# xiangxiecrypto/tfhe-omr

Measured on AMD Instinct MI355X. Metric: detect-phase messages/sec + per-message latency, D=65536 at 1/2/4/8 MI355X, higher is better.
Workload: dtype f64

## Files before the change

tfhe-omr_amd/csrc/br2_fft.hpp:

```cpp
#pragma once

#include "exactness.hpp"
#include "fft1024.hpp"
#include "handoff.hpp"
#include "level2_common.hpp"

namespace omr {

__device__ __forceinline__ int key_pos(int t, int e) { return e * Fft1024::T + t; }


struct Digits2S {
  static constexpr int DW = 2;
  static_assert(LOGB2 == 7 && D2 == 6 && DROP2 == 8, "closed form written for the level-2 basis");
  __device__ static __forceinline__ void pack(double v, uint32_t (&pk)[DW]) {
    const double y = floor(__fma_rn(v, 1.0 / 256.0, 0.5)) + (17315143744.0 + 6755399441055744.0);
    const uint64_t b = __builtin_bit_cast(uint64_t, y);
    const uint32_t lo = (uint32_t)b, hi = (uint32_t)(b >> 32);
    pk[0] = lo ^ 0x102040u;
    pk[1] = __builtin_amdgcn_alignbit(hi, lo, 21) ^ 0x2040u;
  }
  static constexpr int TOP_WIDTH = 16;
  template <int H>
  __device__ static __forceinline__ double digit(const uint32_t (&pk)[DW], int j) {
    return (double)(int)__builtin_amdgcn_sbfe(pk[H], 7 * j, H == 1 && j == 2 ? TOP_WIDTH : 7);
  }
};

__device__ __forceinline__ double limb_acc(double acc, double lo, double hr) {
  using M = Mod<2>;
  const double x = acc + lo;
  const double hi = hr * LIMB;
  const double k = rint(__fma_rn(hr, LIMB * M::QINV, x * M::QINV));
  return canon_small<M>(__fma_rn(-k, M::Q, hi) + x);
}

constexpr int BR2_ROW = 4 * Fft1024::n;
__device__ __forceinline__ __amdgpu_buffer_rsrc_t bsk2_rsrc(const double2 *bskf) {
  constexpr uint32_t bytes = (uint32_t)((size_t)NI * 2 * D2 * BR2_ROW * sizeof(double2));
  return __builtin_amdgcn_make_buffer_rsrc(const_cast<double2 *>(bskf), 0, bytes, 0x00020000);
}
typedef unsigned br2_v4u __attribute__((ext_vector_type(4)));
__device__ __forceinline__ void br2f_load_block(double2 (&k)[Fft1024::E], __amdgpu_buffer_rsrc_t rsrc, int q, int o,
                                                int l, uint32_t t16) {
#pragma unroll
  for (int e = 0; e < Fft1024::E; ++e) {
    const uint32_t soff = (uint32_t)q * (uint32_t)(BR2_ROW * sizeof(double2)) +
                          (uint32_t)(((o * 2 + l) * Fft1024::n + e * Fft1024::T) * sizeof(double2));
    k[e] = __builtin_bit_cast(double2, __builtin_amdgcn_raw_buffer_load_b128(rsrc, t16, (int)soff, 0));
  }
}
__device__ __forceinline__ void br2f_load_half(double2 (&k)[2][Fft1024::E], __amdgpu_buffer_rsrc_t rsrc, int q,
                                               int o, uint32_t t16) {
  br2f_load_block(k[0], rsrc, q, o, 0, t16);
  br2f_load_block(k[1], rsrc, q, o, 1, t16);
}
__device__ __forceinline__ void br2f_mac(const double (&xr)[Fft1024::E], const double (&xi)[Fft1024::E],
                                         const double2 (&k)[2][Fft1024::E], double (&sr)[2][Fft1024::E],
                                         double (&si)[2][Fft1024::E]) {
#pragma unroll
  for (int l = 0; l < 2; ++l)
#pragma unroll
    for (int e = 0; e < Fft1024::E; ++e) {
      const double2 kv = k[l][e];
      sr[l][e] = __fma_rn(xr[e], kv.x, __fma_rn(-xi[e], kv.y, sr[l][e]));
      si[l][e] = __fma_rn(xr[e], kv.y, __fma_rn(xi[e], kv.x, si[l][e]));
    }
}
__device__ __forceinline__ void br2f_zero(double (&sr)[2][2][Fft1024::E], double (&si)[2][2][Fft1024::E]) {
#pragma unroll
  for (int o = 0; o < 2; ++o)
#pragma unroll
    for (int l = 0; l < 2; ++l)
#pragma unroll
      for (int e = 0; e < Fft1024::E; ++e) sr[o][l][e] = si[o][l][e] = 0.0;
}

__device__ __forceinline__ void br2f_digits(const double *acp, int a, int t,
                                            uint32_t (&pk)[2][Fft1024::E][Digits2S::DW]) {
  using F = Fft1024;
  using M = Mod<2>;
  constexpr int NN = N2;
#pragma unroll
  for (int h = 0; h < 2; ++h)
#pragma unroll
    for (int e = 0; e < F::E; ++e) {
      const int c = F::idx(0, t, e) + F::n * h;
      const uint32_t u = (uint32_t)(c - a) & (2 * NN - 1);
      const double v = acp[F::slot_stage(u & (NN - 1))];
      const uint32_t vh = (uint32_t)(__builtin_bit_cast(uint64_t, v) >> 32) ^ ((u & NN) << (31 - 11));
      const double rot = __builtin_bit_cast(double, (__builtin_bit_cast(uint64_t, v) & 0xffffffffull) |
                                                        ((uint64_t)vh << 32));
      Digits2S::pack(canon_small<M>(rot - acp[F::slot_stage(c)]), pk[h][e]);
      asm volatile("" : "+v"(pk[h][e][0]), "+v"(pk[h][e][1]));
    }
}

template <int W>
__device__ __forceinline__ void br2f_digit(const uint32_t (&pk)[2][Fft1024::E][Digits2S::DW], int j, int q, int nx,
                                           double (&sr)[2][2][Fft1024::E], double (&si)[2][2][Fft1024::E],
                                           double2 (&ka)[2][Fft1024::E], double2 (&kb)[2][Fft1024::E], double2 *X,
                                           __amdgpu_buffer_rsrc_t rsrc, uint32_t t16, int t, const double2 (&wc)[4][2]) {
  using F = Fft1024;
  constexpr int E = F::E;
  double xr[E], xi[E];
#pragma unroll
  for (int e = 0; e < E; ++e) {
    xr[e] = Digits2S::digit<W>(pk[0][e], j);
    xi[e] = Digits2S::digit<W>(pk[1][e], j);
  }
  constexpr int LE = 1;
  F::fwd(xr, xi, X, t, wc, [&]() {
    __builtin_amdgcn_s_setprio(2);
#pragma unroll
    for (int l = 0; l < LE; ++l) br2f_load_block(kb[l], rsrc, q, 1, l, t16);
  });
#pragma unroll
  for (int l = LE; l < 2; ++l) br2f_load_block(kb[l], rsrc, q, 1, l, t16);
#pragma unroll
  for (int o = 0; o < 2; ++o) {
    br2f_mac(xr, xi, o ? kb : ka, sr[o], si[o]);
    if (o == 0) br2f_load_half(ka, rsrc, nx, 0, t16);
  }
  __builtin_amdgcn_s_setprio(0);
}

template <bool G>
__device__ __forceinline__ void br2f_update(double *aco, const double (&sr)[2][Fft1024::E],
                                           const double (&si)[2][Fft1024::E], RoundGuard<G> &rg, int t) {
  using F = Fft1024;
#pragma unroll
  for (int e = 0; e < F::E; ++e)
#pragma unroll
    for (int h = 0; h < 2; ++h) {
      const double ylo = h ? si[0][e] : sr[0][e], yhi = h ? si[1][e] : sr[1][e];
      const double lo = rint(ylo), hr = rint(yhi);
      rg.note(ylo, lo);
      rg.note(yhi, hr);
      double &a = aco[F::slot_stage(F::idx(0, t, e) + F::n * h)];
      a = limb_acc(a, lo, hr);
    }
}

constexpr size_t BR2_LDS_X = 0, BR2_LDS_TWS = 4 * (size_t)Fft1024::n * sizeof(double2),
                 BR2_LDS_BYTES = BR2_LDS_TWS + (size_t)Fft1024::n * sizeof(double2);
struct Br2Lds {
  double2 *tws;
  double2 (*Xb)[Fft1024::n];
  double *acs;
};
__device__ __forceinline__ Br2Lds br2_lds(double2 *pool) {
  double2 *x = pool + BR2_LDS_X / sizeof(double2);
  return {pool + BR2_LDS_TWS / sizeof(double2), reinterpret_cast<double2(*)[Fft1024::n]>(x),
          reinterpret_cast<double *>(x + 2 * Fft1024::n)};
}

template <bool G>
__device__ __forceinline__ void br2f_trace(const Br2Lds &lds, const double2 *__restrict__ tkf,
                                           const double2 *__restrict__ twg, const DeviceTables &tb,
                                           RoundGuard<G> &rg, int t) {
  using F = Fft1024;
  using M = Mod<2>;
  constexpr int E = F::E, NN = N2;
  double *acs = lds.acs;
  double2(*Xb)[F::n] = lds.Xb;
  const double2 *tws = lds.tws;
  double2 wc[4][2];
  F::load_ct(wc, twg, t);
  static_assert(DT == 25 && TRACE_STEPS == 11, "trace geometry");
#pragma unroll
  for (int p = 0; p < 2; ++p)
#pragma unroll
    for (int h = 0; h < 2; ++h)
#pragma unroll
      for (int e = 0; e < E; ++e) {
        double &x = acs[p * NN + F::slot_stage(F::idx(0, t, e) + F::n * h)];
        x = canon<M>(mm<M>(x, NINV2));
      }
  constexpr uint32_t bytes = (uint32_t)((size_t)TRACE_STEPS * DT * BR2_ROW * sizeof(double2));
  const __amdgpu_buffer_rsrc_t rsrc = __builtin_amdgcn_make_buffer_rsrc(const_cast<double2 *>(tkf), 0, bytes, 0x00020000);
  const uint32_t t16 = (uint32_t)t * 16u;
#pragma unroll 1
  for (int k = 0; k < TRACE_STEPS; ++k) {
    const uint16_t *src = tb.trace_src + k * NN;
    double2 ka[2][E], kb[2][E];
    br2f_load_half(ka, rsrc, k * DT, 0, t16);
    __syncthreads();
    uint32_t pk[2][E][DigitsTrace::DW];
#pragma unroll
    for (int h = 0; h < 2; ++h)
#pragma unroll
      for (int e = 0; e < E; ++e) {
        const int sidx = src[F::idx(0, t, e) + F::n * h];
        const double v = sidx < NN ? acs[F::slot_stage(sidx)] : -acs[F::slot_stage(sidx - NN)];
        DigitsTrace::pack(v, pk[h][e]);
        asm volatile("" : "+v"(pk[h][e][0]), "+v"(pk[h][e][1]));
      }
    double sr[2][2][E], si[2][2][E];
    br2f_zero(sr, si);
#pragma unroll 1
    for (int d = 0; d < DT; ++d) {
      const int q = k * DT + d;
      double xr[E], xi[E];
#pragma unroll
      for (int e = 0; e < E; ++e) {
        xr[e] = DigitsTrace::get(pk[0][e], d);
        xi[e] = DigitsTrace::get(pk[1][e], d);
      }
      F::fwd(xr, xi, Xb[d & 1], t, wc, [&]() { br2f_load_block(kb[0], rsrc, q, 1, 0, t16); });
      br2f_load_block(kb[1], rsrc, q, 1, 1, t16);
#pragma unroll
      for (int o = 0; o < 2; ++o) {
        br2f_mac(xr, xi, o ? kb : ka, sr[o], si[o]);
        if (o == 0) br2f_load_half(ka, rsrc, d + 1 < DT ? q + 1 : q, 0, t16);
      }
    }
#pragma unroll
    for (int o = 0; o < 2; ++o)
#pragma unroll
      for (int l = 0; l < 2; ++l) F::inv(sr[o][l], si[o][l], Xb[l], tws, t);
    double sb[2][E];
    const uint16_t *srcb = src;
#pragma unroll
    for (int h = 0; h < 2; ++h)
#pragma unroll
      for (int e = 0; e < E; ++e) {
        const int sidx = srcb[F::idx(0, t, e) + F::n * h];
        sb[h][e] = sidx < NN ? acs[NN + F::slot_stage(sidx)] : -acs[NN + F::slot_stage(sidx - NN)];
      }
    __syncthreads();
#pragma unroll
    for (int e = 0; e < E; ++e)
#pragma unroll
      for (int h = 0; h < 2; ++h) {
        const int c = F::slot_stage(F::idx(0, t, e) + F::n * h);
        const double alo = h ? si[0][0][e] : sr[0][0][e], ahi = h ? si[0][1][e] : sr[0][1][e];
        const double blo = h ? si[1][0][e] : sr[1][0][e], bhi = h ? si[1][1][e] : sr[1][1][e];
        const double ral = rint(alo), rah = rint(ahi), rbl = rint(blo), rbh = rint(bhi);
        rg.note(alo, ral);
        rg.note(ahi, rah);
        rg.note(blo, rbl);
        rg.note(bhi, rbh);
        acs[c] = limb_acc(acs[c], ral, rah);
        acs[NN + c] = limb_acc(acs[NN + c] + sb[h][e], rbl, rbh);
      }
  }
}

template <bool G, bool FROM = false>
__device__ __forceinline__ void br2f_body(const uint32_t *__restrict__ lwe_int, const double2 *__restrict__ bskf,
                                          const double2 *__restrict__ twg, DeviceTables tb, uint64_t *__restrict__ out,
                                          unsigned long long *margin, double2 *pool, size_t item,
                                          const uint64_t *__restrict__ acc0 = nullptr) {
  using F = Fft1024;
  using M = Mod<2>;
  constexpr int E = F::E, NN = N2;
  static_assert(F::TW_LEN <= F::n, "the twiddle table's LDS doubles as the trace's NTT table");
  const Br2Lds lds = br2_lds(pool);
  double2 *tws = lds.tws;
  double2(*Xb)[F::n] = lds.Xb;
  double *acs = lds.acs;
  const int t = threadIdx.x;
  const uint32_t *lwe = lwe_int + item * (NI + 1);
  F::load_twiddles(tws, twg, t);
  if constexpr (FROM) {
    const uint64_t *a0 = acc0 + item * 2 * NN;
#pragma unroll
    for (int h = 0; h < 2; ++h)
#pragma unroll
      for (int e = 0; e < E; ++e) {
        const int c = F::idx(0, t, e) + F::n * h;
        acs[F::slot_stage(c)] = from_u64<M>(a0[c]);
        acs[NN + F::slot_stage(c)] = from_u64<M>(a0[NN + c]);
      }
  } else {
    const int b = (int)lwe[NI];
#pragma unroll
    for (int h = 0; h < 2; ++h)
#pragma unroll
      for (int e = 0; e < E; ++e) {
        const int c = F::idx(0, t, e) + F::n * h;
        acs[F::slot_stage(c)] = 0.0;
        acs[NN + F::slot_stage(c)] = acc2_init(tb.lut2, b, c);
      }
  }
  __syncthreads();
  double2 wc[4][2];
  F::load_ct(wc, twg, t);
  double2 ka[2][E], kb[2][E];
  const __amdgpu_buffer_rsrc_t rsrc = bsk2_rsrc(bskf);
  const uint32_t t16 = (uint32_t)t * 16u;
  RoundGuard<G> rg;
  int kq = -1;
#pragma unroll 1
  for (int i = 0; i < NI; ++i) {
    const int a = (int)__builtin_amdgcn_readfirstlane(lwe[i]) & (2 * NN - 1);
    if (a == 0) continue;
    const int q0 = i * 2 * D2;
    if (kq != q0) br2f_load_half(ka, rsrc, q0, 0, t16);
    kq = i + 1 < NI ? q0 + 2 * D2 : -1;
    wg_barrier_lds();
    double sr[2][2][E], si[2][2][E];
#pragma unroll
    for (int p = 0; p < 2; ++p) {
      uint32_t pk[2][E][Digits2S::DW];
      br2f_digits(acs + p * NN, a, t, pk);
      auto nxt = [&](int j, int w) {
        return q0 + (w == 0 ? p * D2 + j + 3
                            : (j + 1 < D2 / 2 ? p * D2 + j + 1 : (p == 0 ? D2 : (kq >= 0 ? 2 * D2 : 2 * D2 - 1))));
      };
      if (p == 0) br2f_zero(sr, si);
#pragma unroll 1
      for (int j = 0; j < D2 / 2; ++j) {
        br2f_digit<0>(pk, j, q0 + p * D2 + j, nxt(j, 0), sr, si, ka, kb, Xb[0], rsrc, t16, t, wc);
        br2f_digit<1>(pk, j, q0 + p * D2 + j + 3, nxt(j, 1), sr, si, ka, kb, Xb[1], rsrc, t16, t, wc);
      }
    }
#pragma unroll
    for (int o = 0; o < 2; ++o) {
#pragma unroll
      for (int l = 0; l < 2; ++l) F::inv(sr[o][l], si[o][l], Xb[l], tws, t);
      br2f_update<G>(acs + o * NN, sr[o], si[o], rg, t);
    }
  }
  rg.publish(margin);
  __syncthreads();
  uint64_t *o = out + item * 2 * NN;
#pragma unroll
  for (int p = 0; p < 2; ++p)
#pragma unroll
    for (int h = 0; h < 2; ++h)
#pragma unroll
      for (int e = 0; e < E; ++e) {
        const int c = F::idx(0, t, e) + F::n * h;
        o[p * NN + c] = to_u64<M>(acs[p * NN + F::slot_stage(c)]);
      }
}

template <bool G>
__device__ __forceinline__ void trace_fft_body(uint64_t *__restrict__ io, const double2 *__restrict__ tkf,
                                               const double2 *__restrict__ twg, DeviceTables tb,
                                               unsigned long long *margin) {
  using F = Fft1024;
  using M = Mod<2>;
  constexpr int E = F::E, NN = N2;
  __shared__ double2 pool[BR2_LDS_BYTES / sizeof(double2)];
  const Br2Lds lds = br2_lds(pool);
  double2 *tws = lds.tws;
  double *acs = lds.acs;
  const int t = threadIdx.x;
  uint64_t *o = io + (size_t)blockIdx.x * 2 * NN;
  F::load_twiddles(tws, twg, t);
#pragma unroll
  for (int p = 0; p < 2; ++p)
#pragma unroll
    for (int h = 0; h < 2; ++h)
#pragma unroll
      for (int e = 0; e < E; ++e) {
        const int c = F::idx(0, t, e) + F::n * h;
        acs[p * NN + F::slot_stage(c)] = from_u64<M>(o[p * NN + c]);
      }
  RoundGuard<G> rg;
  br2f_trace<G>(lds, tkf, twg, tb, rg, t);
  rg.publish(margin);
  __syncthreads();
  using NTT = WgNtt<M, BR2_T, BR2_E>;
  double ca[BR2_E], cb[BR2_E];
#pragma unroll
  for (int e = 0; e < BR2_E; ++e) {
    ca[e] = acs[F::slot_stage(t + e * BR2_T)];
    cb[e] = acs[NN + F::slot_stage(t + e * BR2_T)];
  }
  double *xch = reinterpret_cast<double *>(lds.Xb);
  double *tw = reinterpret_cast<double *>(tws);
  static_assert(NTT::LDS_DOUBLES * sizeof(double) <= 2 * F::n * sizeof(double2), "NTT exchange below ACC");
#pragma unroll
  for (int e = 0; e < BR2_E; ++e) tw[t + e * BR2_T] = tb.tw2[t + e * BR2_T];
  __syncthreads();
  NTT::fwd(ca, xch, tw, t);
  NTT::fwd(cb, xch, tw, t);
#pragma unroll
  for (int e = 0; e < BR2_E; ++e) {
    const int j = t * BR2_E + e;
    o[j] = to_u64<M>(canon<M>(ca[e]));
    o[NN + j] = to_u64<M>(canon<M>(cb[e]));
  }
}
#ifndef OMR_LEVEL2_PARTS_ONLY
__global__ __launch_bounds__(256, 2) void trace_fft_kernel(uint64_t *__restrict__ io, const double2 *__restrict__ tkf,
                                                           const double2 *__restrict__ twg, DeviceTables tb) {
  trace_fft_body<false>(io, tkf, twg, tb, nullptr);
}
__global__ __launch_bounds__(256, 2) void trace_fft_guard_kernel(uint64_t *__restrict__ io,
                                                                 const double2 *__restrict__ tkf,
                                                                 const double2 *__restrict__ twg, DeviceTables tb,
                                                                 unsigned long long *margin) {
  trace_fft_body<true>(io, tkf, twg, tb, margin);
}

__global__ __launch_bounds__(256, 2) void br2f_kernel(const uint32_t *__restrict__ lwe_int,
                                                      const double2 *__restrict__ bskf,
                                                      const double2 *__restrict__ twg, DeviceTables tb,
                                                      uint64_t *__restrict__ out) {
  __shared__ double2 pool[BR2_LDS_BYTES / sizeof(double2)];
  br2f_body<false>(lwe_int, bskf, twg, tb, out, nullptr, pool, blockIdx.x);
}
__global__ __launch_bounds__(256, 2) void br2f_guard_kernel(const uint32_t *__restrict__ lwe_int,
                                                            const double2 *__restrict__ bskf,
                                                            const double2 *__restrict__ twg, DeviceTables tb,
                                                            uint64_t *__restrict__ out, unsigned long long *margin) {
  __shared__ double2 pool[BR2_LDS_BYTES / sizeof(double2)];
  br2f_body<true>(lwe_int, bskf, twg, tb, out, margin, pool, blockIdx.x);
}
__global__ __launch_bounds__(256, 2) void br2f_from_kernel(const uint32_t *__restrict__ lwe_int,
                                                           const double2 *__restrict__ bskf,
                                                           const double2 *__restrict__ twg, DeviceTables tb,
                                                           uint64_t *__restrict__ out,
                                                           const uint64_t *__restrict__ acc0) {
  __shared__ double2 pool[BR2_LDS_BYTES / sizeof(double2)];
  br2f_body<false, true>(lwe_int, bskf, twg, tb, out, nullptr, pool, blockIdx.x, acc0);
}
__global__ __launch_bounds__(256, 2) void br2f_guard_from_kernel(const uint32_t *__restrict__ lwe_int,
                                                                 const double2 *__restrict__ bskf,
                                                                 const double2 *__restrict__ twg, DeviceTables tb,
                                                                 uint64_t *__restrict__ out,
                                                                 unsigned long long *margin,
                                                                 const uint64_t *__restrict__ acc0) {
  __shared__ double2 pool[BR2_LDS_BYTES / sizeof(double2)];
  br2f_body<true, true>(lwe_int, bskf, twg, tb, out, margin, pool, blockIdx.x, acc0);
}
#endif


constexpr int BR2Y_T = 2 * Fft1024::T;
constexpr int BR2Y_H = 4, BR2Y_PF = 2;

__device__ __forceinline__ void br2y_prefetch(const uint32_t *__restrict__ lwe_int, const double2 *__restrict__ bskf,
                                              const uint32_t *flags, int wid, int k) {
  constexpr int STEP_LINES = D2 * BR2_ROW * (int)sizeof(double2) / 64;
  constexpr int PER_THREAD = STEP_LINES / (BR2Y_H * BR2Y_T);
  static_assert(PER_THREAD * BR2Y_H * BR2Y_T == STEP_LINES, "helpers split a step's rows evenly");
  __shared__ int go;
  const int m = wid >> 1, r = wid & 1;
  const uint32_t *lwe = lwe_int + (size_t)m * (NI + 1);
  uint32_t acc = 0;
  int e = 0;
#pragma unroll 1
  for (int i = 0; i < NI; ++i) {
    const int a = (int)__builtin_amdgcn_readfirstlane(lwe[i]) & (2 * N2 - 1);
    if (a == 0) continue;
    if (threadIdx.x == 0) {
      int ok = 1, n = 0;
      while ((int)__hip_atomic_load(flags + wid, __ATOMIC_RELAXED, __HIP_MEMORY_SCOPE_AGENT) < e - BR2Y_PF) {
        if (++n == (1 << 16)) {
          ok = 0;
          break;
        }
        __builtin_amdgcn_s_sleep(2);
      }
      go = ok;
    }
    __syncthreads();
    if (!go) break;
    const char *rows = reinterpret_cast<const char *>(bskf + ((size_t)i * 2 * D2 + (size_t)r * D2) * BR2_ROW);
    uint32_t v[PER_THREAD];
#pragma unroll
    for (int u = 0; u < PER_THREAD; ++u)
      v[u] = *reinterpret_cast<const uint32_t *>(rows + (size_t)((u * BR2Y_H + k) * BR2Y_T + (int)threadIdx.x) * 64);
#pragma unroll
    for (int u = 0; u < PER_THREAD; ++u) acc ^= v[u];
    __syncthreads();
    ++e;
  }
  asm volatile("" ::"v"(acc));
}

#ifndef OMR_LEVEL2_PARTS_ONLY
__global__ __launch_bounds__(BR2Y_T, 1) void br2y_kernel(const uint32_t *__restrict__ lwe_int,
                                                         const double2 *__restrict__ bskf,
                                                         const double2 *__restrict__ twg, DeviceTables tb,
                                                         double *xg, uint32_t *flags, int *err,
                                                         uint64_t *__restrict__ out, int nmsg, int w8,
                                                         int allow_fast) {
#define OMR_BR2Y_FROM 0
#include "br2y_kernel_body.inc"
#undef OMR_BR2Y_FROM
}
#endif

}
```

tfhe-omr_amd/csrc/fft1024.hpp:

```cpp
#pragma once

#include "device_fft.hpp"

namespace omr {

struct Fft1024 {
  static constexpr int T = 256, E = 4, n = 1024, L = 10;
  static constexpr int TW_LEN = 3 * (4 + 16 + 64 + 256);
  OMR_HD static constexpr int tw_off(int p) { return p == 1 ? 0 : p == 2 ? 12 : p == 3 ? 60 : 252; }
  static constexpr int CT_LEN = 2 * (4 + 16 + 64 + 256);
  OMR_HD static constexpr int ct_off(int p) { return p == 1 ? 0 : p == 2 ? 8 : p == 3 ? 40 : 168; }

  OMR_HD static constexpr int lay(int p, int k) {
    constexpr int tab[5][10] = {{9, 8, 7, 6, 3, 2, 1, 0, 5, 4},
                                {7, 6, 9, 8, 3, 2, 1, 0, 5, 4},
                                {5, 4, 3, 2, 1, 0, 9, 8, 7, 6},
                                {3, 2, 5, 4, 1, 0, 9, 8, 7, 6},
                                {1, 0, 5, 4, 3, 2, 9, 8, 7, 6}};
    return tab[p][k];
  }
  OMR_HD static constexpr int idx(int p, int t, int e) {
    const int pos[10] = {(e >> 1) & 1, e & 1, (t >> 5) & 1, (t >> 4) & 1, (t >> 3) & 1, (t >> 2) & 1,
                         (t >> 1) & 1, t & 1, (t >> 7) & 1, (t >> 6) & 1};
    int j = 0;
    for (int k = 0; k < 10; ++k) j |= pos[k] << lay(p, k);
    return j;
  }
  OMR_HD static constexpr int bit(int j, int b) { return (j >> b) & 1; }
  OMR_HD static constexpr int slot_xf(int j) {
    return bit(j, 0) | bit(j, 1) << 1 | (bit(j, 2) ^ bit(j, 8)) << 2 | bit(j, 9) << 3 | bit(j, 8) << 4 |
           bit(j, 3) << 5 | ((j >> 4) & 15) << 6;
  }
  OMR_HD static constexpr int slot_xi(int j) {
    return bit(j, 0) | (bit(j, 1) ^ bit(j, 8)) << 1 | (bit(j, 2) ^ bit(j, 9)) << 2 | bit(j, 3) << 3 |
           bit(j, 8) << 4 | bit(j, 9) << 5 | ((j >> 4) & 15) << 6;
  }
  OMR_HD static constexpr int slot_wf(int j) {
    return bit(j, 8) | bit(j, 9) << 1 | (bit(j, 2) ^ bit(j, 0)) << 2 | bit(j, 3) << 3 | bit(j, 0) << 4 |
           bit(j, 1) << 5 | ((j >> 4) & 15) << 6;
  }
  OMR_HD static constexpr int slot_wi(int j) {
    return bit(j, 8) | bit(j, 9) << 1 | (bit(j, 2) ^ bit(j, 0)) << 2 | bit(j, 1) << 3 | bit(j, 0) << 4 |
           bit(j, 3) << 5 | ((j >> 4) & 15) << 6;
  }
  OMR_HD static constexpr int slot_stage(int c) { return c ^ (((c >> 6) & 1) << 4); }

  static constexpr double C8 = 0.92387953251128675613, S8 = 0.38268343236508977173, R2 = 0.70710678118654752440;
  static constexpr double T8 = 0.41421356237309504880;

  __device__ static __forceinline__ void cmulc(double &xr, double &xi, double wr, double wi) {
    const double r = __fma_rn(xr, wr, xi * wi);
    const double i = __fma_rn(xi, wr, -xr * wi);
    xr = r;
    xi = i;
  }
  __device__ static __forceinline__ void inet4(double (&xr)[E], double (&xi)[E]) {
    const double a0r = xr[0] + xr[1], a0i = xi[0] + xi[1], a1r = xr[0] - xr[1], a1i = xi[0] - xi[1];
    const double b0r = xr[2] + xr[3], b0i = xi[2] + xi[3];
    const double b1r = xi[2] - xi[3], b1i = xr[3] - xr[2];
    xr[0] = a0r + b0r;
    xi[0] = a0i + b0i;
    xr[2] = a0r - b0r;
    xi[2] = a0i - b0i;
    xr[1] = a1r + b1r;
    xi[1] = a1i + b1i;
    xr[3] = a1r - b1r;
    xi[3] = a1i - b1i;
  }
  template <int P>
  __device__ static __forceinline__ int block(int t) {
    return idx(P, t, 0) >> (L - 2 * P);
  }
  OMR_HD static constexpr int tw_slot(int P, int b, int k) {
    return P == 3 ? tw_off(3) + k * 64 + (b ^ (((b >> 4) & 3) << 1))
         : P == 4 ? tw_off(4) + k * 256 + (b ^ (((b >> 6) & 3) << 2))
                  : tw_off(P) + 3 * b + k;
  }
  __device__ static __forceinline__ void load_twiddles(double2 *tws, const double2 *__restrict__ twg, int t) {
    for (int j = t; j < TW_LEN; j += T) {
      const int P = j < tw_off(2) ? 1 : j < tw_off(3) ? 2 : j < tw_off(4) ? 3 : 4;
      const int r = j - tw_off(P);
      tws[tw_slot(P, r / 3, r % 3)] = twg[j];
    }
  }
  template <int P>
  __device__ static __forceinline__ void inv_pass(double (&xr)[E], double (&xi)[E], const double2 *tws, int t) {
    inet4(xr, xi);
    if constexpr (P == 0) {
      cmulc(xr[1], xi[1], C8, S8);
      cmulc(xr[2], xi[2], R2, R2);
      cmulc(xr[3], xi[3], S8, C8);
    } else {
      const int b = block<P>(t);
      const double2 B = tws[tw_slot(P, b, 0)], A = tws[tw_slot(P, b, 1)], AB = tws[tw_slot(P, b, 2)];
      cmulc(xr[1], xi[1], B.x, B.y);
      cmulc(xr[2], xi[2], A.x, A.y);
      cmulc(xr[3], xi[3], AB.x, AB.y);
    }
  }
  __device__ static __forceinline__ void inv_pass_w(double (&xr)[E], double (&xi)[E], const double2 (&w)[3]) {
    inet4(xr, xi);
    cmulc(xr[1], xi[1], w[0].x, w[0].y);
    cmulc(xr[2], xi[2], w[1].x, w[1].y);
    cmulc(xr[3], xi[3], w[2].x, w[2].y);
  }
  template <int P>
  __device__ static __forceinline__ void inv_tw(double2 (&w)[3], const double2 *tws, int t) {
    const int b = block<P>(t);
#pragma unroll
    for (int k = 0; k < 3; ++k) w[k] = tws[tw_slot(P, b, k)];
  }
  __device__ static __forceinline__ void perm(double (&xr)[E], double (&xi)[E]) {
    swap_lane_bit<5>(xr[0], xr[2]);
    swap_lane_bit<5>(xi[0], xi[2]);
    swap_lane_bit<5>(xr[1], xr[3]);
    swap_lane_bit<5>(xi[1], xi[3]);
    swap_lane_bit<4>(xr[0], xr[1]);
    swap_lane_bit<4>(xi[0], xi[1]);
    swap_lane_bit<4>(xr[2], xr[3]);
    swap_lane_bit<4>(xi[2], xi[3]);
  }
  OMR_HD static constexpr int swz(int S, int j) {
    return S == 0 ? slot_xf(j) : S == 1 ? slot_xi(j) : S == 2 ? slot_wf(j) : slot_wi(j);
  }
  OMR_HD static constexpr int base_mask(int S, int P) {
    int m = 0;
    for (int t = 0; t < T; ++t) m |= swz(S, idx(P, t, 0));
    return m;
  }
  template <int S, int P>
  __device__ static __forceinline__ int slot_of(int base, int e) {
    constexpr int M0 = base_mask(S, P);
    const int k = swz(S, idx(P, 0, e));
    return (k & M0 ? base ^ (k & M0) : base) + (k & ~M0);
  }
  template <int PF, int PT, int S, bool CROSS>
  __device__ static __forceinline__ void exchange(double (&xr)[E], double (&xi)[E], double2 *buf, int t) {
    const int bw = swz(S, idx(PF, t, 0)), br = swz(S, idx(PT, t, 0));
#pragma unroll
    for (int e = 0; e < E; ++e) buf[slot_of<S, PF>(bw, e)] = make_double2(xr[e], xi[e]);
    if constexpr (CROSS)
      wg_barrier_lds();
    else
      wave_lds_sync();
#pragma unroll
    for (int e = 0; e < E; ++e) {
      const double2 v = buf[slot_of<S, PT>(br, e)];
      xr[e] = v.x;
      xi[e] = v.y;
    }
    wave_lds_fence();
  }
  __device__ static __forceinline__ void fwd_pass_t(double (&xr)[E], double (&xi)[E], double2 A, double2 B) {
    bfly<false>(xr[0], xi[0], xr[2], xi[2], A.x, A.y);
    bfly<false>(xr[1], xi[1], xr[3], xi[3], A.x, A.y);
    bfly<false>(xr[0], xi[0], xr[1], xi[1], B.x, B.y);
    bfly<true>(xr[2], xi[2], xr[3], xi[3], B.x, B.y);
  }
  template <int P>
  __device__ static __forceinline__ void block_ct(double2 (&w)[2], const double2 *__restrict__ twg, int t) {
    const int b = block<P>(t);
#pragma unroll
    for (int k = 0; k < 2; ++k) w[k] = twg[TW_LEN + ct_off(P) + 2 * b + k];
  }
  __device__ static __forceinline__ void load_ct(double2 (&wc)[4][2], const double2 *__restrict__ twg, int t) {
    block_ct<1>(wc[0], twg, t);
    block_ct<2>(wc[1], twg, t);
    block_ct<3>(wc[2], twg, t);
    block_ct<4>(wc[3], twg, t);
  }
  struct NoMid {
    __device__ void operator()() const {}
  };
  template <typename Mid = NoMid>
  __device__ static __forceinline__ void fwd(double (&xr)[E], double (&xi)[E], double2 *X, int t,
                                             const double2 (&wc)[4][2], Mid mid = Mid()) {
    fwd_pass_t(xr, xi, make_double2(R2, 1.0), make_double2(C8, T8));
    perm(xr, xi);
    fwd_pass_t(xr, xi, wc[0][0], wc[0][1]);
    exchange<1, 2, 0, true>(xr, xi, X, t);
    mid();
    fwd_pass_t(xr, xi, wc[1][0], wc[1][1]);
    perm(xr, xi);
    fwd_pass_t(xr, xi, wc[2][0], wc[2][1]);
    exchange<3, 4, 2, false>(xr, xi, X, t);
    fwd_pass_t(xr, xi, wc[3][0], wc[3][1]);
  }
  __device__ static __forceinline__ void inv(double (&xr)[E], double (&xi)[E], double2 *X, const double2 *tws, int t) {
    double2 w4[3], w3[3], w2[3], w1[3];
    inv_tw<4>(w4, tws, t);
    inv_tw<3>(w3, tws, t);
    inv_pass_w(xr, xi, w4);
    exchange<4, 3, 3, false>(xr, xi, X, t);
    inv_tw<2>(w2, tws, t);
    inv_pass_w(xr, xi, w3);
    perm(xr, xi);
    inv_tw<1>(w1, tws, t);
    inv_pass_w(xr, xi, w2);
    exchange<2, 1, 1, true>(xr, xi, X, t);
    __builtin_amdgcn_s_setprio(2);
    inv_pass_w(xr, xi, w1);
    perm(xr, xi);
    inv_pass<0>(xr, xi, tws, t);
    __builtin_amdgcn_s_setprio(0);
  }
};

constexpr double LIMB = 33554432.0;

}
```

Measured before the change: 15230.

## Skip zero-phase digit work on first iteration and simplify coefficient addressing

Adds a constant-offset 'own' addressing scheme so per-thread coefficient and LDS slot indices become a base plus compile-time offsets, verified by a static_assert. On the first blind-rotation iteration from a fresh accumulator, the all-zero first half is skipped by zeroing sums directly and starting key loads at the second half. The first digit's MAC also initializes accumulators instead of adding to zeros, and the digit loop is re-ordered. The prefetch split inside the forward FFT changes so both key blocks are loaded mid-FFT, which raises register pressure.

```diff
diff --git a/tfhe-omr_amd/csrc/br2_fft.hpp b/tfhe-omr_amd/csrc/br2_fft.hpp
--- a/tfhe-omr_amd/csrc/br2_fft.hpp
+++ b/tfhe-omr_amd/csrc/br2_fft.hpp
@@ -55,6 +55,7 @@
   br2f_load_block(k[0], rsrc, q, o, 0, t16);
   br2f_load_block(k[1], rsrc, q, o, 1, t16);
 }
+template <bool FIRST = false>
 __device__ __forceinline__ void br2f_mac(const double (&xr)[Fft1024::E], const double (&xi)[Fft1024::E],
                                          const double2 (&k)[2][Fft1024::E], double (&sr)[2][Fft1024::E],
                                          double (&si)[2][Fft1024::E]) {
@@ -63,8 +64,13 @@
 #pragma unroll
     for (int e = 0; e < Fft1024::E; ++e) {
       const double2 kv = k[l][e];
-      sr[l][e] = __fma_rn(xr[e], kv.x, __fma_rn(-xi[e], kv.y, sr[l][e]));
-      si[l][e] = __fma_rn(xr[e], kv.y, __fma_rn(xi[e], kv.x, si[l][e]));
+      if constexpr (FIRST) {
+        sr[l][e] = __fma_rn(xr[e], kv.x, -xi[e] * kv.y);
+        si[l][e] = __fma_rn(xr[e], kv.y, xi[e] * kv.x);
+      } else {
+        sr[l][e] = __fma_rn(xr[e], kv.x, __fma_rn(-xi[e], kv.y, sr[l][e]));
+        si[l][e] = __fma_rn(xr[e], kv.y, __fma_rn(xi[e], kv.x, si[l][e]));
+      }
     }
 }
 __device__ __forceinline__ void br2f_zero(double (&sr)[2][2][Fft1024::E], double (&si)[2][2][Fft1024::E]) {
@@ -76,27 +82,31 @@
       for (int e = 0; e < Fft1024::E; ++e) sr[o][l][e] = si[o][l][e] = 0.0;
 }
 
+template <bool OWN = false>
 __device__ __forceinline__ void br2f_digits(const double *acp, int a, int t,
                                             uint32_t (&pk)[2][Fft1024::E][Digits2S::DW]) {
   using F = Fft1024;
   using M = Mod<2>;
   constexpr int NN = N2;
+  const int s0 = F::slot_stage(F::idx(0, t, 0));
+  int ca = F::idx(0, t, 0) - a;
+  if constexpr (OWN) asm volatile("" : "+v"(ca));
 #pragma unroll
   for (int h = 0; h < 2; ++h)
 #pragma unroll
     for (int e = 0; e < F::E; ++e) {
       const int c = F::idx(0, t, e) + F::n * h;
-      const uint32_t u = (uint32_t)(c - a) & (2 * NN - 1);
+      const uint32_t u = (uint32_t)(OWN ? ca + F::own(e, h) : c - a) & (2 * NN - 1);
       const double v = acp[F::slot_stage(u & (NN - 1))];
       const uint32_t vh = (uint32_t)(__builtin_bit_cast(uint64_t, v) >> 32) ^ ((u & NN) << (31 - 11));
       const double rot = __builtin_bit_cast(double, (__builtin_bit_cast(uint64_t, v) & 0xffffffffull) |
                                                         ((uint64_t)vh << 32));
-      Digits2S::pack(canon_small<M>(rot - acp[F::slot_stage(c)]), pk[h][e]);
+      Digits2S::pack(canon_small<M>(rot - acp[OWN ? s0 + F::own(e, h) : F::slot_stage(c)]), pk[h][e]);
       asm volatile("" : "+v"(pk[h][e][0]), "+v"(pk[h][e][1]));
     }
 }
 
-template <int W>
+template <int W, bool FIRST = false>
 __device__ __forceinline__ void br2f_digit(const uint32_t (&pk)[2][Fft1024::E][Digits2S::DW], int j, int q, int nx,
                                            double (&sr)[2][2][Fft1024::E], double (&si)[2][2][Fft1024::E],
                                            double2 (&ka)[2][Fft1024::E], double2 (&kb)[2][Fft1024::E], double2 *X,
@@ -109,7 +119,7 @@
     xr[e] = Digits2S::digit<W>(pk[0][e], j);
     xi[e] = Digits2S::digit<W>(pk[1][e], j);
   }
-  constexpr int LE = 1;
+  constexpr int LE = 2;
   F::fwd(xr, xi, X, t, wc, [&]() {
     __builtin_amdgcn_s_setprio(2);
 #pragma unroll
@@ -119,7 +129,7 @@
   for (int l = LE; l < 2; ++l) br2f_load_block(kb[l], rsrc, q, 1, l, t16);
 #pragma unroll
   for (int o = 0; o < 2; ++o) {
-    br2f_mac(xr, xi, o ? kb : ka, sr[o], si[o]);
+    br2f_mac<FIRST>(xr, xi, o ? kb : ka, sr[o], si[o]);
     if (o == 0) br2f_load_half(ka, rsrc, nx, 0, t16);
   }
   __builtin_amdgcn_s_setprio(0);
@@ -137,7 +147,7 @@
       const double lo = rint(ylo), hr = rint(yhi);
       rg.note(ylo, lo);
       rg.note(yhi, hr);
-      double &a = aco[F::slot_stage(F::idx(0, t, e) + F::n * h)];
+      double &a = aco[F::slot_stage(F::idx(0, t, 0)) + F::own(e, h)];
       a = limb_acc(a, lo, hr);
     }
 }
@@ -261,6 +271,7 @@
   double2(*Xb)[F::n] = lds.Xb;
   double *acs = lds.acs;
   const int t = threadIdx.x;
+  const int c0 = F::idx(0, t, 0), s0 = F::slot_stage(c0);
   const uint32_t *lwe = lwe_int + item * (NI + 1);
   F::load_twiddles(tws, twg, t);
   if constexpr (FROM) {
@@ -269,9 +280,9 @@
     for (int h = 0; h < 2; ++h)
 #pragma unroll
       for (int e = 0; e < E; ++e) {
-        const int c = F::idx(0, t, e) + F::n * h;
-        acs[F::slot_stage(c)] = from_u64<M>(a0[c]);
-        acs[NN + F::slot_stage(c)] = from_u64<M>(a0[NN + c]);
+        const int c = c0 + F::own(e, h);
+        acs[s0 + F::own(e, h)] = from_u64<M>(a0[c]);
+        acs[NN + s0 + F::own(e, h)] = from_u64<M>(a0[NN + c]);
       }
   } else {
     const int b = (int)lwe[NI];
@@ -279,9 +290,8 @@
     for (int h = 0; h < 2; ++h)
 #pragma unroll
       for (int e = 0; e < E; ++e) {
-        const int c = F::idx(0, t, e) + F::n * h;
-        acs[F::slot_stage(c)] = 0.0;
-        acs[NN + F::slot_stage(c)] = acc2_init(tb.lut2, b, c);
+        acs[s0 + F::own(e, h)] = 0.0;
+        acs[NN + s0 + F::own(e, h)] = acc2_init(tb.lut2, b, c0 + F::own(e, h));
       }
   }
   __syncthreads();
@@ -297,23 +307,37 @@
     const int a = (int)__builtin_amdgcn_readfirstlane(lwe[i]) & (2 * NN - 1);
     if (a == 0) continue;
     const int q0 = i * 2 * D2;
-    if (kq != q0) br2f_load_half(ka, rsrc, q0, 0, t16);
+    const bool mask0 = !FROM && kq < 0;
+    if (kq != q0) br2f_load_half(ka, rsrc, mask0 ? q0 + D2 : q0, 0, t16);
     kq = i + 1 < NI ? q0 + 2 * D2 : -1;
     wg_barrier_lds();
     double sr[2][2][E], si[2][2][E];
 #pragma unroll
     for (int p = 0; p < 2; ++p) {
+      if (p == 0 && mask0) {
+        br2f_zero(sr, si);
+        continue;
+      }
       uint32_t pk[2][E][Digits2S::DW];
-      br2f_digits(acs + p * NN, a, t, pk);
+      br2f_digits<true>(acs + p * NN, a, t, pk);
       auto nxt = [&](int j, int w) {
         return q0 + (w == 0 ? p * D2 + j + 3
                             : (j + 1 < D2 / 2 ? p * D2 + j + 1 : (p == 0 ? D2 : (kq >= 0 ? 2 * D2 : 2 * D2 - 1))));
       };
-      if (p == 0) br2f_zero(sr, si);
+      if (p == 0) {
+        br2f_digit<0, true>(pk, 0, q0, nxt(0, 0), sr, si, ka, kb, Xb[0], rsrc, t16, t, wc);
 #pragma unroll 1
-      for (int j = 0; j < D2 / 2; ++j) {
-        br2f_digit<0>(pk, j, q0 + p * D2 + j, nxt(j, 0), sr, si, ka, kb, Xb[0], rsrc, t16, t, wc);
-        br2f_digit<1>(pk, j, q0 + p * D2 + j + 3, nxt(j, 1), sr, si, ka, kb, Xb[1], rsrc, t16, t, wc);
+        for (int j = 0; j < D2 / 2 - 1; ++j) {
+          br2f_digit<1>(pk, j, q0 + j + 3, nxt(j, 1), sr, si, ka, kb, Xb[1], rsrc, t16, t, wc);
+          br2f_digit<0>(pk, j + 1, q0 + j + 1, nxt(j + 1, 0), sr, si, ka, kb, Xb[0], rsrc, t16, t, wc);
+        }
+        br2f_digit<1>(pk, 2, q0 + 5, nxt(2, 1), sr, si, ka, kb, Xb[1], rsrc, t16, t, wc);
+      } else {
+#pragma unroll 1
+        for (int j = 0; j < D2 / 2; ++j) {
+          br2f_digit<0>(pk, j, q0 + p * D2 + j, nxt(j, 0), sr, si, ka, kb, Xb[0], rsrc, t16, t, wc);
+          br2f_digit<1>(pk, j, q0 + p * D2 + j + 3, nxt(j, 1), sr, si, ka, kb, Xb[1], rsrc, t16, t, wc);
+        }
       }
     }
 #pragma unroll
@@ -332,8 +356,7 @@
     for (int h = 0; h < 2; ++h)
 #pragma unroll
       for (int e = 0; e < E; ++e) {
-        const int c = F::idx(0, t, e) + F::n * h;
-        o[p * NN + c] = to_u64<M>(acs[p * NN + F::slot_stage(c)]);
+        o[p * NN + c0 + F::own(e, h)] = to_u64<M>(acs[p * NN + s0 + F::own(e, h)]);
       }
 }
 
diff --git a/tfhe-omr_amd/csrc/fft1024.hpp b/tfhe-omr_amd/csrc/fft1024.hpp
--- a/tfhe-omr_amd/csrc/fft1024.hpp
+++ b/tfhe-omr_amd/csrc/fft1024.hpp
@@ -44,6 +44,16 @@
            bit(j, 3) << 5 | ((j >> 4) & 15) << 6;
   }
   OMR_HD static constexpr int slot_stage(int c) { return c ^ (((c >> 6) & 1) << 4); }
+  OMR_HD static constexpr int own(int e, int h) { return 256 * e + n * h; }
+  OMR_HD static constexpr bool own_ok() {
+    for (int t = 0; t < T; ++t)
+      for (int e = 0; e < E; ++e)
+        for (int h = 0; h < 2; ++h) {
+          const int c = idx(0, t, e) + n * h;
+          if (c != idx(0, t, 0) + own(e, h) || slot_stage(c) != slot_stage(idx(0, t, 0)) + own(e, h)) return false;
+        }
+    return true;
+  }
 
   static constexpr double C8 = 0.92387953251128675613, S8 = 0.38268343236508977173, R2 = 0.70710678118654752440;
   static constexpr double T8 = 0.41421356237309504880;
@@ -206,6 +216,8 @@
   }
 };
 
+static_assert(Fft1024::own_ok(), "own coefficients and their slots at constant offsets");
+
 constexpr double LIMB = 33554432.0;
 
 }
```

After: 15270, median of 3. About the same (+0.3%).
